# huangnengCSU/NanoSNP

Measured on NVIDIA B200. Metric: candidate sites/sec (s1+s2), higher is better.
Workload: dtype int32 counts, fp64 AF gate, fp16 hi/lo split x3 tensor-core model (fp32 accumulate)

## Files before the change

### nanosnp_b200/csrc/model_tc.cu

```cuda
#include <cuda_fp16.h>
#include <stdlib.h>
#include "model_common.cuh"
#include "tc_ptx.cuh"

namespace nsnp {
namespace {

constexpr int kRows = 128;
constexpr float kLog2e = 1.4426950408889634f;

__device__ __forceinline__ uint4 scale_hi(const uint4& hi) {
    const __half2 k = __float2half2_rn(1.0f / kTcLoScale);
    auto m = [&](uint32_t x) { __half2 t = *reinterpret_cast<__half2*>(&x); return h2_bits(__hmul2(t, k)); };
    return make_uint4(m(hi.x), m(hi.y), m(hi.z), m(hi.w));
}

template <int LAYER> struct TcCfg;
template <> struct TcCfg<0> { static constexpr int K = kTcK0, IN = kTcIn0, STEPS = 33; };
template <> struct TcCfg<1> { static constexpr int K = kTcK1, IN = kTcIn1, STEPS = 17; };

template <int LAYER, int CG> struct TcSmem {
    static constexpr int K = TcCfg<LAYER>::K;
    static constexpr int RB = 256 / CG;
    static constexpr size_t b_bytes = (size_t)K * RB * 2;
    static constexpr size_t a_bytes = (size_t)K * kRows * 2;
    static constexpr size_t sc_bytes = LAYER == 0 ? (size_t)kTcIn0 * kRows * 2 : 0;
    static constexpr size_t off_bhi = 0, off_blo = b_bytes, off_ahi = 2 * b_bytes, off_alo = off_ahi + a_bytes,
                            off_asc = off_alo + a_bytes, off_bar = off_asc + sc_bytes, off_bias = off_bar + 64,
                            total = off_bias + (LAYER == 1 ? 256 * sizeof(float) : 0);
};

template <int LAYER, int CG, int NWQ, bool DEBUG>
__global__ void __launch_bounds__(128 * NWQ + (LAYER == 1 ? 32 : 0), (LAYER == 0 && CG == 2 && NWQ == 2) ? 2 : 1)
lstm_tc_kernel(const unsigned char* __restrict__ blob, const int32_t* __restrict__ xi, const float* __restrict__ xf,
               const __half* __restrict__ h0_in, __half* __restrict__ h0_out, float* __restrict__ h16, float* __restrict__ dbg,
               int64_t n, int dir_override)
{
    using C = TcCfg<LAYER>;
    using S = TcSmem<LAYER, CG>;
    constexpr int K = C::K, IN = C::IN, RB = S::RB;
    constexpr int KB = K / 16;
    constexpr int kThreads = 128 * NWQ + (LAYER == 1 ? 32 : 0);
    constexpr int kEpiWarps = 4 * NWQ;
    constexpr int UB = 8 / NWQ;
    constexpr uint32_t LBO_A = kRows * 16, LBO_B = RB * 16, SBO = 128;
    extern __shared__ __align__(1024) unsigned char smem[];
    unsigned char* sBhi = smem + S::off_bhi; unsigned char* sBlo = smem + S::off_blo;
    unsigned char* sAhi = smem + S::off_ahi; unsigned char* sAlo = smem + S::off_alo; unsigned char* sAsc = smem + S::off_asc;
    uint64_t* bar = reinterpret_cast<uint64_t*>(smem + S::off_bar);
    uint32_t* tmem_slot = reinterpret_cast<uint32_t*>(smem + S::off_bar + 32);

    const int tid = threadIdx.x, lane = tid & 31, warp = tid >> 5;
    const bool producer = LAYER == 1 && warp == kEpiWarps;
    const int quad = warp & 3, sub = producer ? 0 : (warp >> 2);
    const int row = quad * 32 + lane;
    const int dir = DEBUG ? dir_override : (int)blockIdx.y;
    const uint32_t cta_rank = CG == 2 ? cluster_ctarank() : 0u;
    const int64_t site0 = (int64_t)blockIdx.x * kRows;
    int64_t site = site0 + row;
    const bool live = site < n;
    if (!live) site = n - 1;

    if (tid == 0) { mbar_init(bar, 1); mbar_init(bar + 1, 1); mbar_init(bar + 2, 1); fence_mbar_init(); }
    if (warp == 0) tmem_alloc<CG>(tmem_slot, LAYER == 1 ? 512 : 256);
    {
        const uint4* ghi = reinterpret_cast<const uint4*>(blob + tc_off(LAYER, dir, 0));
        const uint4* glo = reinterpret_cast<const uint4*>(blob + tc_off(LAYER, dir, 1));
        uint4* dhi = reinterpret_cast<uint4*>(sBhi); uint4* dlo = reinterpret_cast<uint4*>(sBlo);
        for (int i = tid; i < (K / 8) * RB; i += kThreads) {
            const int ch = i / RB, r = i - ch * RB;
            const int g = ch * 256 + (int)cta_rank * RB + r;
            dhi[i] = __ldg(ghi + g); dlo[i] = __ldg(glo + g);
        }
        uint4* a = reinterpret_cast<uint4*>(sAhi);
        const int n16 = (int)((2 * S::a_bytes + S::sc_bytes) / 16);
        for (int i = tid; i < n16; i += kThreads) a[i] = make_uint4(0, 0, 0, 0);
    }
    __syncthreads();
    const float* sBias = reinterpret_cast<const float*>(smem + S::off_bias);
    if (LAYER == 1) {
        const float* gb = reinterpret_cast<const float*>(blob + kOffTcBias1) + dir * 256;
        for (int i = tid; i < 256; i += kThreads) reinterpret_cast<float*>(smem + S::off_bias)[i] = __ldg(gb + i);
        __syncthreads();
    }

    float c[UB][8];
#pragma unroll
    for (int j = 0; j < UB; ++j)
#pragma unroll
        for (int u = 0; u < 8; ++u) c[j][u] = 0.f;

    int2 xraw[8];
    auto load_x = [&](int t) {
        if (LAYER != 0) return;
        const int2* g = reinterpret_cast<const int2*>(xi ? (const void*)(xi + (site * kT + t) * kF) : (const void*)(xf + (site * kT + t) * kF));
        if (sub == 0) {
#pragma unroll
            for (int j = 0; j < 8; ++j) xraw[j] = ldg_nc_volatile(g + j);
        } else if (sub == NWQ - 1) {
            xraw[0] = ldg_nc_volatile(g + 8);
        }
    };
    auto xval = [&](int j) -> float {
        const int2 p = xraw[j >> 1];
        const int b = (j & 1) ? p.y : p.x;
        return xi ? (float)b : __int_as_float(b);
    };
    auto store_x = [&]() {
        if (LAYER != 0) return;
        if (sub == 0) {
#pragma unroll
            for (int ch = 0; ch < 2; ++ch) {
                float v[8];
#pragma unroll
                for (int j = 0; j < 8; ++j) v[j] = xval(ch * 8 + j);
                const HiLo8 s = split8(v);
                reinterpret_cast<uint4*>(sAhi + ch * LBO_A)[row] = s.hi;
                reinterpret_cast<uint4*>(sAlo + ch * LBO_A)[row] = s.lo;
                reinterpret_cast<uint4*>(sAsc + ch * LBO_A)[row] = scale_hi(s.hi);
            }
        } else if (sub == NWQ - 1) {
            const float v[8] = {xval(0), xval(1), 1.0f, 0.f, 0.f, 0.f, 0.f, 0.f};
            const HiLo8 s = split8(v);
            reinterpret_cast<uint4*>(sAhi + 2 * LBO_A)[row] = s.hi;
            reinterpret_cast<uint4*>(sAlo + 2 * LBO_A)[row] = s.lo;
            reinterpret_cast<uint4*>(sAsc + 2 * LBO_A)[row] = scale_hi(s.hi);
        }
    };
    uint64_t* barS = bar + 2;
    constexpr uint32_t kPartBytes = 16u * kRows * 16u;
    const bool l2_prefetch = (dir_override >> 8) & 1;
    const int npass = ((dir_override >> 16) & 3) ? ((dir_override >> 16) & 3) : 3;
    const size_t src_tile = min((size_t)blockIdx.x, (size_t)((n + kRows - 1) / kRows - 1));
    auto stage_h0_bulk = [&](int t) {
        const __half* src = h0_in + (src_tile * kT + t) * (2 * kPartBytes / 2);
        mbar_expect_tx(barS, 2 * kPartBytes);
        bulk_g2s(sAhi, src, kPartBytes, barS);
        bulk_g2s(sAlo, src + kPartBytes / 2, kPartBytes, barS);
        const int tp = dir == 0 ? t + 1 : t - 1;
        if (l2_prefetch && tp >= 0 && tp < kT) bulk_prefetch_l2(h0_in + (src_tile * kT + tp) * (2 * kPartBytes / 2), 2 * kPartBytes);
    };
    constexpr int XB = IN / 16;
    constexpr uint32_t kTmemCols = LAYER == 1 ? 512 : 256;
    uint64_t* barH = bar;
    uint64_t* barX = bar + 1;
    {
        const int t0 = dir == 0 ? 0 : kT - 1;
        load_x(t0); store_x();
        fence_async_smem();
    }

    tc_fence_before();
    if (CG == 2) cluster_sync_all(); else __syncthreads();
    tc_fence_after();
    uint32_t phaseH = 0, phaseX = 0, phaseS = 0;
    if (LAYER == 1) {
        if (producer && lane == 0) stage_h0_bulk(dir == 0 ? 0 : kT - 1);
        mbar_wait(barS, phaseS); phaseS ^= 1;
        tc_fence_before();
        if (CG == 2) cluster_sync_all(); else __syncthreads();
        tc_fence_after();
    }
    const uint32_t tmem_base = *tmem_slot;
    const uint32_t a_hi = smem_u32(sAhi), a_lo = smem_u32(sAlo), a_sc = smem_u32(sAsc), b_hi = smem_u32(sBhi), b_lo = smem_u32(sBlo);
    constexpr uint32_t idesc = make_idesc(128 * CG, 256);
    const bool issuer = cta_rank == 0 && tid == 0;
    auto issue = [&](int kb0, int kb1, uint32_t tmem_d, uint32_t acc) {
#pragma unroll 1
        for (int pass = 0; pass < npass; ++pass) {
#pragma unroll 1
            for (int kb = kb0; kb < kb1; ++kb) {
                uint32_t aa = pass == 2 ? a_lo : a_hi;
                if (LAYER == 0 && pass == 1 && kb < kTcIn0 / 16) aa = a_sc;
                const uint32_t bb = pass == 1 ? b_lo : b_hi;
                umma_f16<CG>(tmem_d, make_desc(aa + kb * 2 * LBO_A, LBO_A, SBO), make_desc(bb + kb * 2 * LBO_B, LBO_B, SBO), idesc, acc);
                acc = 1;
            }
        }
    };
    if (LAYER == 1) {
        if (issuer) { tc_fence_after(); issue(0, XB, tmem_base, 0); umma_commit<CG>(barX); }
        if (producer) {
            mbar_wait(barX, phaseX); phaseX ^= 1;
            if (lane == 0 && C::STEPS > 1 && !DEBUG) stage_h0_bulk(dir == 0 ? 1 : kT - 2);
        }
    }

    for (int step = 0; step < C::STEPS; ++step) {
        const int t = dir == 0 ? step : (kT - 1 - step);
        const int tn = dir == 0 ? step + 1 : (kT - 2 - step);
        const bool more = !DEBUG && step + 1 < C::STEPS;
        const uint32_t acc_cols = LAYER == 1 ? (uint32_t)(step & 1) * 256u : 0u;
        if (LAYER == 1 && more) { mbar_wait(barS, phaseS); phaseS ^= 1; }
        fence_async_smem();
        tc_fence_before();
        if (CG == 2) cluster_sync_exec(); else __syncthreads();
        if (issuer) {
            tc_fence_after();
            if (LAYER == 1) {
                issue(XB, KB, tmem_base + acc_cols, 1);
                umma_commit<CG>(barH);
                if (more) { issue(0, XB, tmem_base + (acc_cols ^ 256u), 0); umma_commit<CG>(barX); }
            } else {
                issue(0, KB, tmem_base, 0);
                umma_commit<CG>(barH);
            }
        }
        if (producer) {
            if (more) {
                mbar_wait(barX, phaseX); phaseX ^= 1;
                if (lane == 0 && step + 2 < C::STEPS) stage_h0_bulk(dir == 0 ? step + 2 : kT - 3 - step);
            }
            if (DEBUG) break;
            continue;
        }
        if (more) load_x(tn);
        mbar_wait(barH, phaseH);
        phaseH ^= 1;
        tc_fence_after();

        if (DEBUG) {
#pragma unroll 1
            for (int jb = sub * UB; jb < sub * UB + UB; ++jb) {
                float v[32];
                tmem_ld32(tmem_base + acc_cols + ((uint32_t)(quad * 32) << 16) + jb * 32, v);
                if (live) for (int i = 0; i < 32; ++i) dbg[(site0 + row) * 256 + jb * 32 + i] = v[i] + (LAYER == 1 ? sBias[jb * 32 + i] : 0.f);
            }
            break;
        }

        uint32_t vb[2][16];
        const uint32_t tacc = tmem_base + acc_cols + ((uint32_t)(quad * 32) << 16) + (uint32_t)(sub * UB) * 32u;
        tmem_ld16_nowait(tacc, vb[0]);
        tmem_wait_ld();
        float hv[8];
#pragma unroll
        for (int hb = 0; hb < 2 * UB; ++hb) {
            const int jl = hb >> 1, uh = hb & 1, jb = sub * UB + jl;
            if (hb + 1 < 2 * UB) tmem_ld16_nowait(tacc + (hb + 1) * 16, vb[(hb + 1) & 1]);
#pragma unroll
            for (int u = 0; u < 4; ++u) {
                const uint32_t* v = vb[hb & 1];
                const float* bq = sBias + jb * 32 + uh * 16 + u;
                const float bi_ = LAYER == 1 ? bq[0] : 0.f, bf_ = LAYER == 1 ? bq[4] : 0.f, bg_ = LAYER == 1 ? bq[8] : 0.f, bo_ = LAYER == 1 ? bq[12] : 0.f;
                const float xi_ = fminf(__uint_as_float(v[u]) + bi_, 36.f), xf_ = fminf(__uint_as_float(v[4 + u]) + bf_, 36.f);
                const float xg_ = fminf(__uint_as_float(v[8 + u]) + bg_, 36.f), xo_ = __uint_as_float(v[12 + u]) + bo_;
                const float ei = ex2_approx(xi_), ef = ex2_approx(xf_), eg = ex2_approx(xg_), eo = ex2_approx(xo_);
                const float pi = 1.f + ei, pf = 1.f + ef, pg = 1.f + eg;
                const float pig = pi * pg;
                const float num = fmaf(c[jl][uh * 4 + u], pig, fmaf(eg, 2.f * kLog2e, -2.f * kLog2e) * pf);
                const float cn = num * rcp_approx(pf * pig);
                c[jl][uh * 4 + u] = cn;
                const float ec = ex2_approx(cn);
                hv[uh * 4 + u] = (1.f - ec) * rcp_approx((1.f + eo) * (1.f + ec));
            }
            if (hb + 1 < 2 * UB) tmem_wait_ld();
            if (uh == 1) {
                const HiLo8 s = split8(hv);
                reinterpret_cast<uint4*>(sAhi + (IN / 8 + jb) * LBO_A)[row] = s.hi;
                reinterpret_cast<uint4*>(sAlo + (IN / 8 + jb) * LBO_A)[row] = s.lo;
                if (live) {
                    if (LAYER == 0) {
                        __half* o = h0_out + ((((size_t)blockIdx.x * kT + t) * 2) * 16 + (dir * 8 + jb)) * (kRows * 8) + row * 8;
                        *reinterpret_cast<uint4*>(o) = s.hi;
                        *reinterpret_cast<uint4*>(o + 16 * kRows * 8) = s.lo;
                    } else if (step == C::STEPS - 1) {
                        float4* o = reinterpret_cast<float4*>(h16 + site * 128 + dir * kH + jb * 8);
                        o[0] = make_float4(hv[0], hv[1], hv[2], hv[3]); o[1] = make_float4(hv[4], hv[5], hv[6], hv[7]);
                    }
                }
            }
        }
        if (more) store_x();
    }

    tc_fence_before();
    if (CG == 2) cluster_sync_all(); else __syncthreads();
    if (warp == 0) tmem_dealloc<CG>(tmem_base, kTmemCols);
}


__device__ __forceinline__ void mbar_arrive(uint64_t* bar) {
    asm volatile("mbarrier.arrive.shared::cta.b64 _, [%0];" ::"r"(smem_u32(bar)) : "memory");
}

constexpr int kP2GroupThreads = 256, kP2Threads = 2 * kP2GroupThreads;
struct P2Smem {
    static constexpr size_t b_bytes = (size_t)kTcK0 * 128 * 2;
    static constexpr size_t a_bytes = (size_t)kTcK0 * kRows * 2;
    static constexpr size_t sc_bytes = (size_t)kTcIn0 * kRows * 2;
    static constexpr size_t a_stride = 2 * a_bytes + sc_bytes;
    static constexpr size_t off_bhi = 0, off_blo = b_bytes, off_a = 2 * b_bytes, off_bar = off_a + 2 * a_stride, total = off_bar + 128;
};

__global__ void __launch_bounds__(kP2Threads, 1)
lstm0_pair2_kernel(const unsigned char* __restrict__ blob, const int32_t* __restrict__ xi, const float* __restrict__ xf,
                   __half* __restrict__ h0_out, int64_t n, const int32_t* __restrict__ pos, int64_t pos_bias, int npass)
{
    using S = P2Smem;
// ... 325 lines not shown
                const float xi_ = fminf(__uint_as_float(v[u]) + bq[0], 36.f), xf_ = fminf(__uint_as_float(v[4 + u]) + bq[4], 36.f);
                const float xg_ = fminf(__uint_as_float(v[8 + u]) + bq[8], 36.f), xo_ = __uint_as_float(v[12 + u]) + bq[12];
                const float ei = ex2_approx(xi_), ef = ex2_approx(xf_), eg = ex2_approx(xg_), eo = ex2_approx(xo_);
                const float pi = 1.f + ei, pf = 1.f + ef, pg = 1.f + eg;
                const float pig = pi * pg;
                const float num = fmaf(c[jl][uh * 4 + u], pig, fmaf(eg, 2.f * kLog2e, -2.f * kLog2e) * pf);
                const float cn = num * rcp_approx(pf * pig);
                c[jl][uh * 4 + u] = cn;
                const float ec = ex2_approx(cn);
                hv[uh * 4 + u] = (1.f - ec) * rcp_approx((1.f + eo) * (1.f + ec));
            }
            if (hb + 1 < 2 * UB) tmem_wait_ld();
            if (uh == 1) {
                const HiLo8 sp = split8(hv);
                reinterpret_cast<uint4*>(sA + (IN / 8 + jb) * LBO_A)[row] = sp.hi;
                if (live && step == kS - 1) {
                    float4* o = reinterpret_cast<float4*>(h16 + site * 128 + dir * kH + jb * 8);
                    o[0] = make_float4(hv[0], hv[1], hv[2], hv[3]); o[1] = make_float4(hv[4], hv[5], hv[6], hv[7]);
                }
            }
        }
        if (more) {
            if (warp == 0) { mbar_wait(barIn, phaseIn); phaseIn ^= 1; }
            report_ready();
        }
        if (++step == kS) { step = 0; ++qi; }
    }

    tc_fence_before();
    cluster_sync_all();
    if (threadIdx.x < 32) tmem_dealloc<2>(*tmem_slot, 512);
}

template <class Kern, class... Args>
int launch_pair2(Kern kern, const char* name, size_t smem_bytes, int64_t m, cudaStream_t stream, Args... args) {
    const unsigned quads = (unsigned)((m + 4 * kRows - 1) / (4 * kRows));
    unsigned clusters = 2 * quads; if (clusters > (unsigned)kNumSMs / 2) clusters = ((unsigned)kNumSMs / 2) & ~1u;
    cudaLaunchConfig_t cfg = {};
    cfg.gridDim = dim3(2 * clusters, 1, 1);
    cfg.blockDim = dim3(kP2Threads, 1, 1);
    cfg.dynamicSmemBytes = smem_bytes;
    cfg.stream = stream;
    cudaLaunchAttribute attr[1];
    attr[0].id = cudaLaunchAttributeClusterDimension;
    attr[0].val.clusterDim.x = 2; attr[0].val.clusterDim.y = 1; attr[0].val.clusterDim.z = 1;
    cfg.attrs = attr; cfg.numAttrs = 1;
    const cudaError_t e = cudaLaunchKernelEx(&cfg, kern, args...);
    if (e != cudaSuccess) return set_error(NSNP_E_CUDA, "%s: %s", name, cudaGetErrorString(e));
    return NSNP_OK;
}

int launch_l0_pair2(const void* blob, const int32_t* xi, const float* xf, void* h0_out, int64_t m, const int32_t* pos, int64_t pos_bias, int npass, cudaStream_t stream) {
    static bool attr_done = false;
    if (!attr_done) {
        if (cudaFuncSetAttribute(lstm0_pair2_kernel, cudaFuncAttributeMaxDynamicSharedMemorySize, (int)P2Smem::total) != cudaSuccess)
            return cuda_status("cudaFuncSetAttribute(lstm0_pair2_kernel)");
        attr_done = true;
    }
    return launch_pair2(lstm0_pair2_kernel, "lstm0_pair2_kernel", P2Smem::total, m, stream, (const unsigned char*)blob, xi, xf, (__half*)h0_out, m, pos, pos_bias, npass);
}

int launch_l1_pair2(const void* blob, const void* h0_in, float* h16, int64_t m, cudaStream_t stream) {
    static bool attr_done = false;
    if (!attr_done) {
        if (cudaFuncSetAttribute(lstm1_pair2_kernel, cudaFuncAttributeMaxDynamicSharedMemorySize, (int)P2Smem1::total) != cudaSuccess)
            return cuda_status("cudaFuncSetAttribute(lstm1_pair2_kernel)");
        attr_done = true;
    }
    return launch_pair2(lstm1_pair2_kernel, "lstm1_pair2_kernel", P2Smem1::total, m, stream, (const unsigned char*)blob, (const __half*)h0_in, h16, m);
}

constexpr int kTtEpiWarps = 8, kTtLoadWarps = 4;
constexpr int kTtThreads = (kTtEpiWarps + kTtLoadWarps + 1) * 32;
struct TailSmem {
    static constexpr size_t w_bytes = kTcBytesTail;
    static constexpr size_t a_bytes = (size_t)128 * kRows * 2;
    static constexpr size_t off_whi = 0, off_wlo = w_bytes, off_ahi = 2 * w_bytes, off_alo = off_ahi + a_bytes,
                            off_head = off_alo + a_bytes,
                            off_bias = off_head + 256 * 24 * 4,
                            off_xch = off_bias + (256 + 32) * 4,
                            off_bar = off_xch + 128 * 12 * 4, total = off_bar + 64;
};

__device__ __forceinline__ void named_bar_sync(int id, int nthreads) { asm volatile("bar.sync %0, %1;" ::"r"(id), "r"(nthreads) : "memory"); }

__global__ void __launch_bounds__(kTtThreads, 1)
tail_tc_kernel(const unsigned char* __restrict__ blob, const float* __restrict__ h16, int64_t n_max, const int32_t* __restrict__ n_dev,
               float* __restrict__ gt, float* __restrict__ zy)
{
    using S = TailSmem;
    constexpr uint32_t LBO_A = kRows * 16, LBO_B = 256 * 16, SBO = 128;
    extern __shared__ __align__(1024) unsigned char smem[];
    unsigned char* sWhi = smem + S::off_whi; unsigned char* sWlo = smem + S::off_wlo;
    unsigned char* sAhi = smem + S::off_ahi; unsigned char* sAlo = smem + S::off_alo;
    float* sHead = reinterpret_cast<float*>(smem + S::off_head);
    float* sBias = reinterpret_cast<float*>(smem + S::off_bias);
    float* sXch = reinterpret_cast<float*>(smem + S::off_xch);
    uint64_t* bar = reinterpret_cast<uint64_t*>(smem + S::off_bar);
    uint32_t* tmem_slot = reinterpret_cast<uint32_t*>(smem + S::off_bar + 48);
    uint64_t* barH = bar; uint64_t* barIn = bar + 2; uint64_t* barFree = bar + 3;

    const int tid = threadIdx.x, lane = tid & 31, warp = tid >> 5;
// ... 131 lines not shown
            if (half == 0 && site < n) {
                float m = lg[0];
#pragma unroll
                for (int j = 1; j < 21; ++j) m = fmaxf(m, lg[j]);
                float sum = 0.f;
#pragma unroll
                for (int j = 0; j < 21; ++j) { lg[j] = expf(lg[j] - m); sum += lg[j]; }
#pragma unroll
                for (int j = 0; j < 21; ++j) gt[site * 21 + j] = lg[j] / sum;
                const float m2 = fmaxf(lg[21], fmaxf(lg[22], lg[23]));
                const float e0 = expf(lg[21] - m2), e1 = expf(lg[22] - m2), e2 = expf(lg[23] - m2);
                const float s2 = e0 + e1 + e2;
                zy[site * 3 + 0] = e0 / s2; zy[site * 3 + 1] = e1 / s2; zy[site * 3 + 2] = e2 / s2;
            }
        }
    }

    tc_fence_before();
    __syncthreads();
    if (warp == 0) tmem_dealloc<1>(tmem_base, 512);
}

template <int LAYER, int CG, int NWQ, bool DEBUG>
int launch_one(const void* blob, const int32_t* xi, const float* xf, const void* h0_in, void* h0_out, float* h16, float* dbg,
               int64_t m, int dir_override, cudaStream_t stream)
{
    using S = TcSmem<LAYER, CG>;
    auto kern = lstm_tc_kernel<LAYER, CG, NWQ, DEBUG>;
    static bool attr_done = false;
    if (!attr_done) {
        if (cudaFuncSetAttribute(kern, cudaFuncAttributeMaxDynamicSharedMemorySize, (int)S::total) != cudaSuccess) return cuda_status("cudaFuncSetAttribute(lstm_tc_kernel)");
        attr_done = true;
    }
    unsigned gx = (unsigned)((m + kRows - 1) / kRows);
    if (CG == 2 && (gx & 1)) ++gx;
    cudaLaunchConfig_t cfg = {};
    cfg.gridDim = dim3(gx, DEBUG ? 1 : 2, 1);
    cfg.blockDim = dim3(128 * NWQ + (LAYER == 1 ? 32 : 0), 1, 1);
    cfg.dynamicSmemBytes = S::total;
    cfg.stream = stream;
    cudaLaunchAttribute attr[1];
    attr[0].id = cudaLaunchAttributeClusterDimension;
    attr[0].val.clusterDim.x = CG; attr[0].val.clusterDim.y = 1; attr[0].val.clusterDim.z = 1;
    cfg.attrs = attr; cfg.numAttrs = 1;
    const cudaError_t e = cudaLaunchKernelEx(&cfg, kern, (const unsigned char*)blob, xi, xf, (const __half*)h0_in, (__half*)h0_out, h16, dbg, m, dir_override);
    if (e != cudaSuccess) return set_error(NSNP_E_CUDA, "lstm_tc_kernel<%d,%d,%d>: %s", LAYER, CG, NWQ, cudaGetErrorString(e));
    return NSNP_OK;
}

}

int launch_tail_tc(const void* blob, const float* h16, int64_t n_max, const int32_t* n_dev, float* gt, float* zy, cudaStream_t stream) {
    using S = TailSmem;
    static bool attr_done = false;
    if (!attr_done) {
        if (cudaFuncSetAttribute(tail_tc_kernel, cudaFuncAttributeMaxDynamicSharedMemorySize, (int)S::total) != cudaSuccess)
            return cuda_status("cudaFuncSetAttribute(tail_tc_kernel)");
        attr_done = true;
    }
    const int64_t n_tiles = (n_max + kRows - 1) / kRows;
    const int grid = (int)(n_tiles < kNumSMs ? n_tiles : kNumSMs);
    tail_tc_kernel<<<grid, kTtThreads, S::total, stream>>>((const unsigned char*)blob, h16, n_max, n_dev, gt, zy);
    return cuda_status("tail_tc_kernel");
}

int launch_lstm_tc(const void* blob, const int32_t* xi, const float* xf, void* h0, float* h16, int64_t m, const int32_t* pos, int64_t pos_bias, int npass, cudaStream_t stream) {
    {
        ProfScope prof(NSNP_PROF_LSTM0, stream);
        static const int variant = [] { const char* v = getenv("NSNP_L0_VARIANT"); return v ? atoi(v) : 1; }();
        if (pos && variant != 1) return set_error(NSNP_E_UNSUPPORTED, "window reads from the count tensor need the default layer-0 kernel");
        if (int e = variant == 1 ? launch_l0_pair2(blob, xi, xf, h0, m, pos, pos_bias, npass, stream)
                                 : launch_one<0, 2, 2, false>(blob, xi, xf, nullptr, h0, nullptr, nullptr, m, npass << 16, stream)) return e;
    }
    ProfScope prof(NSNP_PROF_LSTM1, stream);
    static const int pf = [] { const char* v = getenv("NSNP_L1_PREFETCH"); return v ? atoi(v) : 1; }();
    static const int l1_variant = [] { const char* v = getenv("NSNP_L1_VARIANT"); return v ? atoi(v) : 1; }();
    if (npass == 1 && l1_variant == 1) return launch_l1_pair2(blob, h0, h16, m, stream);
    return launch_one<1, 2, 4, false>(blob, nullptr, nullptr, h0, nullptr, h16, nullptr, m, (pf << 8) | (npass << 16), stream);
}

int debug_tc_gates(const void* blob, const int32_t* xi, int layer, int dir, int cg, const void* h0, float* gates_out, int64_t m, cudaStream_t stream) {
    if (layer == 0 && cg == 1) return launch_one<0, 1, 2, true>(blob, xi, nullptr, nullptr, nullptr, nullptr, gates_out, m, dir, stream);
    if (layer == 0 && cg == 2) return launch_one<0, 2, 2, true>(blob, xi, nullptr, nullptr, nullptr, nullptr, gates_out, m, dir, stream);
    if (layer == 1 && cg == 2) return launch_one<1, 2, 4, true>(blob, nullptr, nullptr, h0, nullptr, nullptr, gates_out, m, dir, stream);
    return set_error(NSNP_E_UNSUPPORTED, "debug_tc_gates: layer %d with cta_group %d is not built", layer, cg);
}

int pack_tc_weights(const nsnp_model_weights_t* w, unsigned char* blob) {
    for (int layer = 0; layer < 2; ++layer) {
        const int K = layer == 0 ? kTcK0 : kTcK1, IN = layer == 0 ? kTcIn0 : kTcIn1, nin = layer == 0 ? kF : 128;
        for (int d = 0; d < 2; ++d) {
            __half* hi = reinterpret_cast<__half*>(blob + tc_off(layer, d, 0));
            __half* lo = reinterpret_cast<__half*>(blob + tc_off(layer, d, 1));
            const float *wih = w->w_ih[layer][d], *whh = w->w_hh[layer][d], *bi = w->b_ih[layer][d], *bh = w->b_hh[layer][d];
            for (int n = 0; n < 256; ++n) {
                const int jb = n >> 5, uh = (n >> 4) & 1, gate = (n >> 2) & 3, u4 = n & 3;
                const int rowi = gate * kH + jb * 8 + uh * 4 + u4;
                for (int k = 0; k < K; ++k) {
                    float v = 0.f;
                    if (k < nin) v = wih[rowi * nin + k];
                    else if (layer == 0 && k == nin) v = bi[rowi] + bh[rowi];
                    else if (k >= IN) v = whh[rowi * kH + (k - IN)];
                    v *= gate == 2 ? -2.0f * kLog2e : -kLog2e;
                    const float scale = (layer == 0 && k < IN) ? kTcLoScale : 1.0f;
                    const __half h = __float2half_rn(v);
                    const __half l = __float2half_rn((v - __half2float(h)) * scale);
                    const size_t idx = ((size_t)(k >> 3) * 256 + n) * 8 + (k & 7);
                    hi[idx] = h; lo[idx] = l;
                }
                if (layer == 1) reinterpret_cast<float*>(blob + kOffTcBias1)[d * 256 + n] = (bi[rowi] + bh[rowi]) * (gate == 2 ? -2.0f * kLog2e : -kLog2e);
// ... 28 lines not shown
```

### nanosnp_b200/csrc/tc_ptx.cuh

```cuda
#pragma once
#include <cuda_fp16.h>
#include <stdint.h>

namespace nsnp {
namespace {

__device__ __forceinline__ uint32_t smem_u32(const void* p) { return (uint32_t)__cvta_generic_to_shared(p); }
__device__ __forceinline__ void mbar_init(uint64_t* bar, uint32_t count) {
    asm volatile("mbarrier.init.shared::cta.b64 [%0], %1;" ::"r"(smem_u32(bar)), "r"(count) : "memory");
}
__device__ __forceinline__ void fence_mbar_init() { asm volatile("fence.mbarrier_init.release.cluster;" ::: "memory"); }
__device__ __forceinline__ void mbar_wait(uint64_t* bar, uint32_t parity) {
    asm volatile(
        "{\n\t.reg .pred P1;\n\t"
        "WAIT_LOOP:\n\t"
        "mbarrier.try_wait.parity.shared::cta.b64 P1, [%0], %1;\n\t"
        "@P1 bra DONE;\n\t"
        "bra WAIT_LOOP;\n\t"
        "DONE:\n\t}"
        ::"r"(smem_u32(bar)), "r"(parity) : "memory");
}
__device__ __forceinline__ void mbar_wait_cluster(uint64_t* bar, uint32_t parity) {
    asm volatile(
        "{\n\t.reg .pred P1;\n\t"
        "WAIT_LOOP_C:\n\t"
        "mbarrier.try_wait.parity.acquire.cluster.shared::cta.b64 P1, [%0], %1;\n\t"
        "@P1 bra DONE_C;\n\t"
        "bra WAIT_LOOP_C;\n\t"
        "DONE_C:\n\t}"
        ::"r"(smem_u32(bar)), "r"(parity) : "memory");
}
__device__ __forceinline__ void mbar_arrive_remote_relaxed(uint64_t* bar, uint32_t target_cta) {
    uint32_t raddr;
    asm volatile("mapa.shared::cluster.u32 %0, %1, %2;" : "=r"(raddr) : "r"(smem_u32(bar)), "r"(target_cta));
    asm volatile("mbarrier.arrive.relaxed.cluster.shared::cluster.b64 _, [%0];" ::"r"(raddr) : "memory");
}
__device__ __forceinline__ void fence_async_smem() { asm volatile("fence.proxy.async.shared::cta;" ::: "memory"); }
__device__ __forceinline__ void tc_fence_before() { asm volatile("tcgen05.fence::before_thread_sync;" ::: "memory"); }
__device__ __forceinline__ void tc_fence_after() { asm volatile("tcgen05.fence::after_thread_sync;" ::: "memory"); }
__device__ __forceinline__ void cluster_sync_all() {
    asm volatile("barrier.cluster.arrive.release.aligned;\n\tbarrier.cluster.wait.acquire.aligned;" ::: "memory");
}
__device__ __forceinline__ void cluster_sync_exec() {
    asm volatile("barrier.cluster.arrive.relaxed.aligned;\n\tbarrier.cluster.wait.aligned;" ::: "memory");
}
__device__ __forceinline__ uint32_t cluster_ctarank() { uint32_t r; asm volatile("mov.u32 %0, %%cluster_ctarank;" : "=r"(r)); return r; }

template <int CG> __device__ __forceinline__ void tmem_alloc(uint32_t* dst_smem, uint32_t ncols) {
    if (CG == 1) {
        asm volatile("tcgen05.alloc.cta_group::1.sync.aligned.shared::cta.b32 [%0], %1;" ::"r"(smem_u32(dst_smem)), "r"(ncols) : "memory");
        asm volatile("tcgen05.relinquish_alloc_permit.cta_group::1.sync.aligned;" ::: "memory");
    } else {
        asm volatile("tcgen05.alloc.cta_group::2.sync.aligned.shared::cta.b32 [%0], %1;" ::"r"(smem_u32(dst_smem)), "r"(ncols) : "memory");
        asm volatile("tcgen05.relinquish_alloc_permit.cta_group::2.sync.aligned;" ::: "memory");
    }
}
template <int CG> __device__ __forceinline__ void tmem_dealloc(uint32_t taddr, uint32_t ncols) {
    if (CG == 1) asm volatile("tcgen05.dealloc.cta_group::1.sync.aligned.b32 %0, %1;" ::"r"(taddr), "r"(ncols) : "memory");
    else asm volatile("tcgen05.dealloc.cta_group::2.sync.aligned.b32 %0, %1;" ::"r"(taddr), "r"(ncols) : "memory");
}
template <int CG> __device__ __forceinline__ void umma_f16(uint32_t tmem_d, uint64_t adesc, uint64_t bdesc, uint32_t idesc, uint32_t accumulate) {
    if (CG == 1)
        asm volatile("{\n\t.reg .pred p;\n\tsetp.ne.b32 p, %4, 0;\n\ttcgen05.mma.cta_group::1.kind::f16 [%0], %1, %2, %3, p;\n\t}"
                     ::"r"(tmem_d), "l"(adesc), "l"(bdesc), "r"(idesc), "r"(accumulate) : "memory");
    else
        asm volatile("{\n\t.reg .pred p;\n\tsetp.ne.b32 p, %4, 0;\n\ttcgen05.mma.cta_group::2.kind::f16 [%0], %1, %2, %3, p;\n\t}"
                     ::"r"(tmem_d), "l"(adesc), "l"(bdesc), "r"(idesc), "r"(accumulate) : "memory");
}
// ... 79 lines not shown
```

Measured before the change: 41.58 million.

## Make layer-1 LSTM kernel persistent with cross-tile pipelined input GEMM and cluster barrier

Layer 1 now launches a persistent grid capped at the SM count. Each cluster loops over several 128-row tiles for one direction and resets the cell state at each tile boundary. The h0 bulk staging and the input-projection MMA are pipelined across tile boundaries, so the next tile's first step overlaps with the current tile's last step. A new cluster-scope mbarrier lets the rank-0 issuer, now the producer warp, wait until both CTAs have staged their inputs. This is meant to remove per-tile launch, TMEM allocation and weight-load overhead and to keep the tensor core busy. The cost is more complex phase tracking and fewer resident CTAs when there are few tiles.

Result: faster. 42.08 million, median of 6 (+1.2%).

```diff
diff --git a/nanosnp_b200/csrc/model_tc.cu b/nanosnp_b200/csrc/model_tc.cu
--- a/nanosnp_b200/csrc/model_tc.cu
+++ b/nanosnp_b200/csrc/model_tc.cu
@@ -40,6 +40,7 @@
     using S = TcSmem<LAYER, CG>;
     constexpr int K = C::K, IN = C::IN, RB = S::RB;
     constexpr int KB = K / 16;
+    constexpr int kS = DEBUG ? 1 : C::STEPS;
     constexpr int kThreads = 128 * NWQ + (LAYER == 1 ? 32 : 0);
     constexpr int kEpiWarps = 4 * NWQ;
     constexpr int UB = 8 / NWQ;
@@ -54,14 +55,31 @@
     const bool producer = LAYER == 1 && warp == kEpiWarps;
     const int quad = warp & 3, sub = producer ? 0 : (warp >> 2);
     const int row = quad * 32 + lane;
-    const int dir = DEBUG ? dir_override : (int)blockIdx.y;
     const uint32_t cta_rank = CG == 2 ? cluster_ctarank() : 0u;
-    const int64_t site0 = (int64_t)blockIdx.x * kRows;
-    int64_t site = site0 + row;
-    const bool live = site < n;
-    if (!live) site = n - 1;
-
-    if (tid == 0) { mbar_init(bar, 1); mbar_init(bar + 1, 1); mbar_init(bar + 2, 1); fence_mbar_init(); }
+    int dir, unit0, unit_stride = 0, my_tiles = 1;
+    if (LAYER == 1) {
+        const int cluster = (int)blockIdx.x / CG, n_clusters = (int)gridDim.x / CG;
+        const int n_units = (int)((n + CG * kRows - 1) / (CG * kRows));
+        dir = DEBUG ? dir_override : cluster & 1;
+        unit0 = DEBUG ? cluster : cluster >> 1;
+        unit_stride = DEBUG ? n_clusters : n_clusters >> 1;
+        my_tiles = (n_units - unit0 + unit_stride - 1) / unit_stride;
+    } else {
+        dir = DEBUG ? dir_override : (int)blockIdx.y;
+        unit0 = (int)blockIdx.x / CG;
+    }
+    const int total = my_tiles * kS;
+    auto tile_of = [&](int qi) -> int64_t { return (int64_t)(unit0 + qi * unit_stride) * CG + cta_rank; };
+    int64_t tile = LAYER == 1 ? tile_of(0) : (int64_t)blockIdx.x, site;
+    bool live;
+    auto enter_tile = [&]() {
+        site = tile * kRows + row;
+        live = site < n;
+        if (!live) site = n - 1;
+    };
+    enter_tile();
+
+    if (tid == 0) { mbar_init(bar, 1); mbar_init(bar + 1, 1); mbar_init(bar + 2, 1); mbar_init(bar + 3, CG); fence_mbar_init(); }
     if (warp == 0) tmem_alloc<CG>(tmem_slot, LAYER == 1 ? 512 : 256);
     {
         const uint4* ghi = reinterpret_cast<const uint4*>(blob + tc_off(LAYER, dir, 0));
@@ -84,12 +102,6 @@
         __syncthreads();
     }
 
-    float c[UB][8];
-#pragma unroll
-    for (int j = 0; j < UB; ++j)
-#pragma unroll
-        for (int u = 0; u < 8; ++u) c[j][u] = 0.f;
-
     int2 xraw[8];
     auto load_x = [&](int t) {
         if (LAYER != 0) return;
@@ -131,19 +143,23 @@
     constexpr uint32_t kPartBytes = 16u * kRows * 16u;
     const bool l2_prefetch = (dir_override >> 8) & 1;
     const int npass = ((dir_override >> 16) & 3) ? ((dir_override >> 16) & 3) : 3;
-    const size_t src_tile = min((size_t)blockIdx.x, (size_t)((n + kRows - 1) / kRows - 1));
-    auto stage_h0_bulk = [&](int t) {
-        const __half* src = h0_in + (src_tile * kT + t) * (2 * kPartBytes / 2);
+    auto h0_rows = [&](int e) -> const __half* {
+        if (e >= total) return nullptr;
+        const int qi = e / kS, st = e - qi * kS;
+        const size_t src_tile = min((size_t)tile_of(qi), (size_t)((n + kRows - 1) / kRows - 1));
+        return h0_in + (src_tile * kT + (dir == 0 ? st : kT - 1 - st)) * (2 * kPartBytes / 2);
+    };
+    auto stage_h0_bulk = [&](const __half* src, const __half* next) {
         mbar_expect_tx(barS, 2 * kPartBytes);
         bulk_g2s(sAhi, src, kPartBytes, barS);
         bulk_g2s(sAlo, src + kPartBytes / 2, kPartBytes, barS);
-        const int tp = dir == 0 ? t + 1 : t - 1;
-        if (l2_prefetch && tp >= 0 && tp < kT) bulk_prefetch_l2(h0_in + (src_tile * kT + tp) * (2 * kPartBytes / 2), 2 * kPartBytes);
+        if (l2_prefetch && next) bulk_prefetch_l2(next, 2 * kPartBytes);
     };
     constexpr int XB = IN / 16;
     constexpr uint32_t kTmemCols = LAYER == 1 ? 512 : 256;
     uint64_t* barH = bar;
     uint64_t* barX = bar + 1;
+    uint64_t* barIn = bar + 3;
     {
         const int t0 = dir == 0 ? 0 : kT - 1;
         load_x(t0); store_x();
@@ -153,10 +169,9 @@
     tc_fence_before();
     if (CG == 2) cluster_sync_all(); else __syncthreads();
     tc_fence_after();
-    uint32_t phaseH = 0, phaseX = 0, phaseS = 0;
     if (LAYER == 1) {
-        if (producer && lane == 0) stage_h0_bulk(dir == 0 ? 0 : kT - 1);
-        mbar_wait(barS, phaseS); phaseS ^= 1;
+        if (producer && lane == 0) stage_h0_bulk(h0_rows(0), h0_rows(1));
+        mbar_wait(barS, 0);
         tc_fence_before();
         if (CG == 2) cluster_sync_all(); else __syncthreads();
         tc_fence_after();
@@ -164,7 +179,7 @@
     const uint32_t tmem_base = *tmem_slot;
     const uint32_t a_hi = smem_u32(sAhi), a_lo = smem_u32(sAlo), a_sc = smem_u32(sAsc), b_hi = smem_u32(sBhi), b_lo = smem_u32(sBlo);
     constexpr uint32_t idesc = make_idesc(128 * CG, 256);
-    const bool issuer = cta_rank == 0 && tid == 0;
+    const bool issuer = cta_rank == 0 && tid == (LAYER == 1 ? kEpiWarps * 32 : 0);
     auto issue = [&](int kb0, int kb1, uint32_t tmem_d, uint32_t acc) {
 #pragma unroll 1
         for (int pass = 0; pass < npass; ++pass) {
@@ -181,42 +196,52 @@
     if (LAYER == 1) {
         if (issuer) { tc_fence_after(); issue(0, XB, tmem_base, 0); umma_commit<CG>(barX); }
         if (producer) {
-            mbar_wait(barX, phaseX); phaseX ^= 1;
-            if (lane == 0 && C::STEPS > 1 && !DEBUG) stage_h0_bulk(dir == 0 ? 1 : kT - 2);
-        }
-    }
-
-    for (int step = 0; step < C::STEPS; ++step) {
-        const int t = dir == 0 ? step : (kT - 1 - step);
-        const int tn = dir == 0 ? step + 1 : (kT - 2 - step);
-        const bool more = !DEBUG && step + 1 < C::STEPS;
-        const uint32_t acc_cols = LAYER == 1 ? (uint32_t)(step & 1) * 256u : 0u;
-        if (LAYER == 1 && more) { mbar_wait(barS, phaseS); phaseS ^= 1; }
+            mbar_wait(barX, 0);
+            if (lane == 0 && total > 1) stage_h0_bulk(h0_rows(1), h0_rows(2));
+        }
+    }
+
+    float c[UB][8];
+    for (int g = 0; g < total; ++g) {
+        const int qi = LAYER == 1 ? g / kS : 0, st = g - qi * kS;
+        const int t = dir == 0 ? st : (kT - 1 - st);
+        const int tn = dir == 0 ? st + 1 : (kT - 2 - st);
+        const bool more = g + 1 < total;
+        const uint32_t acc_cols = LAYER == 1 ? (uint32_t)(g & 1) * 256u : 0u;
+        if (st == 0) {
+            if (g > 0) { tile = tile_of(qi); enter_tile(); }
+#pragma unroll
+            for (int j = 0; j < UB; ++j)
+#pragma unroll
+                for (int u = 0; u < 8; ++u) c[j][u] = 0.f;
+        }
         fence_async_smem();
         tc_fence_before();
         if (CG == 2) cluster_sync_exec(); else __syncthreads();
-        if (issuer) {
-            tc_fence_after();
-            if (LAYER == 1) {
-                issue(XB, KB, tmem_base + acc_cols, 1);
-                umma_commit<CG>(barH);
-                if (more) { issue(0, XB, tmem_base + (acc_cols ^ 256u), 0); umma_commit<CG>(barX); }
-            } else {
-                issue(0, KB, tmem_base, 0);
-                umma_commit<CG>(barH);
-            }
-        }
-        if (producer) {
+        if (LAYER == 0) {
+            if (issuer) { tc_fence_after(); issue(0, KB, tmem_base, 0); umma_commit<CG>(barH); }
+        } else if (producer) {
+            if (issuer) { tc_fence_after(); issue(XB, KB, tmem_base + acc_cols, 1); umma_commit<CG>(barH); }
             if (more) {
-                mbar_wait(barX, phaseX); phaseX ^= 1;
-                if (lane == 0 && step + 2 < C::STEPS) stage_h0_bulk(dir == 0 ? step + 2 : kT - 3 - step);
-            }
-            if (DEBUG) break;
+                const __half* src = h0_rows(g + 2);
+                const __half* next = h0_rows(g + 3);
+                if (lane == 0) {
+                    mbar_wait(barS, (uint32_t)(g + 1) & 1u);
+                    mbar_arrive_remote_release(barIn, 0);
+                }
+                if (issuer) {
+                    mbar_wait_cluster(barIn, (uint32_t)g & 1u);
+                    tc_fence_after();
+                    issue(0, XB, tmem_base + (acc_cols ^ 256u), 0);
+                    umma_commit<CG>(barX);
+                }
+                mbar_wait(barX, (uint32_t)(g + 1) & 1u);
+                if (lane == 0 && src) stage_h0_bulk(src, next);
+            }
             continue;
         }
         if (more) load_x(tn);
-        mbar_wait(barH, phaseH);
-        phaseH ^= 1;
+        mbar_wait(barH, (uint32_t)g & 1u);
         tc_fence_after();
 
         if (DEBUG) {
@@ -224,9 +249,9 @@
             for (int jb = sub * UB; jb < sub * UB + UB; ++jb) {
                 float v[32];
                 tmem_ld32(tmem_base + acc_cols + ((uint32_t)(quad * 32) << 16) + jb * 32, v);
-                if (live) for (int i = 0; i < 32; ++i) dbg[(site0 + row) * 256 + jb * 32 + i] = v[i] + (LAYER == 1 ? sBias[jb * 32 + i] : 0.f);
-            }
-            break;
+                if (live) for (int i = 0; i < 32; ++i) dbg[site * 256 + jb * 32 + i] = v[i] + (LAYER == 1 ? sBias[jb * 32 + i] : 0.f);
+            }
+            continue;
         }
 
         uint32_t vb[2][16];
@@ -257,14 +282,15 @@
             if (hb + 1 < 2 * UB) tmem_wait_ld();
             if (uh == 1) {
                 const HiLo8 s = split8(hv);
-                reinterpret_cast<uint4*>(sAhi + (IN / 8 + jb) * LBO_A)[row] = s.hi;
-                reinterpret_cast<uint4*>(sAlo + (IN / 8 + jb) * LBO_A)[row] = s.lo;
+                const bool h_zero = LAYER == 1 && st == kS - 1;
+                reinterpret_cast<uint4*>(sAhi + (IN / 8 + jb) * LBO_A)[row] = h_zero ? make_uint4(0, 0, 0, 0) : s.hi;
+                reinterpret_cast<uint4*>(sAlo + (IN / 8 + jb) * LBO_A)[row] = h_zero ? make_uint4(0, 0, 0, 0) : s.lo;
                 if (live) {
                     if (LAYER == 0) {
-                        __half* o = h0_out + ((((size_t)blockIdx.x * kT + t) * 2) * 16 + (dir * 8 + jb)) * (kRows * 8) + row * 8;
+                        __half* o = h0_out + ((((size_t)tile * kT + t) * 2) * 16 + (dir * 8 + jb)) * (kRows * 8) + row * 8;
                         *reinterpret_cast<uint4*>(o) = s.hi;
                         *reinterpret_cast<uint4*>(o + 16 * kRows * 8) = s.lo;
-                    } else if (step == C::STEPS - 1) {
+                    } else if (st == kS - 1) {
                         float4* o = reinterpret_cast<float4*>(h16 + site * 128 + dir * kH + jb * 8);
                         o[0] = make_float4(hv[0], hv[1], hv[2], hv[3]); o[1] = make_float4(hv[4], hv[5], hv[6], hv[7]);
                     }
@@ -889,10 +915,16 @@
         if (cudaFuncSetAttribute(kern, cudaFuncAttributeMaxDynamicSharedMemorySize, (int)S::total) != cudaSuccess) return cuda_status("cudaFuncSetAttribute(lstm_tc_kernel)");
         attr_done = true;
     }
-    unsigned gx = (unsigned)((m + kRows - 1) / kRows);
+    unsigned gx = (unsigned)((m + kRows - 1) / kRows), gy = DEBUG ? 1 : 2;
     if (CG == 2 && (gx & 1)) ++gx;
+    if (LAYER == 1) {
+        const unsigned units = gx / CG, cap = ((unsigned)kNumSMs / CG) & ~1u;
+        unsigned clusters = DEBUG ? units : 2 * units;
+        if (clusters > cap) clusters = cap;
+        gx = clusters * CG; gy = 1;
+    }
     cudaLaunchConfig_t cfg = {};
-    cfg.gridDim = dim3(gx, DEBUG ? 1 : 2, 1);
+    cfg.gridDim = dim3(gx, gy, 1);
     cfg.blockDim = dim3(128 * NWQ + (LAYER == 1 ? 32 : 0), 1, 1);
     cfg.dynamicSmemBytes = S::total;
     cfg.stream = stream;
diff --git a/nanosnp_b200/csrc/tc_ptx.cuh b/nanosnp_b200/csrc/tc_ptx.cuh
--- a/nanosnp_b200/csrc/tc_ptx.cuh
+++ b/nanosnp_b200/csrc/tc_ptx.cuh
@@ -34,6 +34,11 @@
     uint32_t raddr;
     asm volatile("mapa.shared::cluster.u32 %0, %1, %2;" : "=r"(raddr) : "r"(smem_u32(bar)), "r"(target_cta));
     asm volatile("mbarrier.arrive.relaxed.cluster.shared::cluster.b64 _, [%0];" ::"r"(raddr) : "memory");
+}
+__device__ __forceinline__ void mbar_arrive_remote_release(uint64_t* bar, uint32_t target_cta) {
+    uint32_t raddr;
+    asm volatile("mapa.shared::cluster.u32 %0, %1, %2;" : "=r"(raddr) : "r"(smem_u32(bar)), "r"(target_cta));
+    asm volatile("mbarrier.arrive.release.cluster.shared::cluster.b64 _, [%0];" ::"r"(raddr) : "memory");
 }
 __device__ __forceinline__ void fence_async_smem() { asm volatile("fence.proxy.async.shared::cta;" ::: "memory"); }
 __device__ __forceinline__ void tc_fence_before() { asm volatile("tcgen05.fence::before_thread_sync;" ::: "memory"); }
```

## Add warp-specialized paired-CTA layer-1 LSTM kernel for three-pass hi/lo split

Applied to the files above, without the earlier changes.

Adds a new layer-1 LSTM kernel for the three-pass (hi/lo split) path. It uses 2-CTA clusters and a dedicated producer warp that streams hi and lo input halves through separate full/empty mbarriers, and it ping-pongs two tile groups on the tensor core. Before this, the npass==3 case fell back to the generic launch_one kernel. The aim is to overlap input loading and the recurrent epilogue with UMMA work and to share weights across the CTA pair. In exchange it adds considerable synchronization complexity, and the input buffer is single-buffered per half, which may stall.

New measurement: 41.15 million before, 43.34 million after, median of 6. +5.3%, better.

```diff
diff --git a/nanosnp_b200/csrc/model_tc.cu b/nanosnp_b200/csrc/model_tc.cu
--- a/nanosnp_b200/csrc/model_tc.cu
+++ b/nanosnp_b200/csrc/model_tc.cu
@@ -656,13 +656,234 @@
     if (threadIdx.x < 32) tmem_dealloc<2>(*tmem_slot, 512);
 }
 
+constexpr int kP2x3Threads = kP2Threads + 32;
+struct P2Smem1x3 {
+    static constexpr size_t b_bytes = (size_t)kTcK1 * 128 * 2;
+    static constexpr size_t in_bytes = (size_t)kTcIn1 * kRows * 2;
+    static constexpr size_t h_bytes = (size_t)kH * kRows * 2;
+    static constexpr size_t off_bhi = 0, off_blo = b_bytes, off_in = 2 * b_bytes, off_h = off_in + 2 * in_bytes,
+                            off_bias = off_h + 4 * h_bytes, off_bar = off_bias + 256 * sizeof(float), total = off_bar + 128;
+};
+static_assert(P2Smem1x3::total <= 232448, "lstm1_pair2x3_kernel: shared memory above the per-block opt-in limit");
+
+__global__ void __launch_bounds__(kP2x3Threads, 1)
+lstm1_pair2x3_kernel(const unsigned char* __restrict__ blob, const __half* __restrict__ h0_in, float* __restrict__ h16, int64_t n)
+{
+    using S = P2Smem1x3;
+    constexpr int K = kTcK1, IN = kTcIn1, KB = K / 16, XB = IN / 16, RB = 128, UB = 4, kS = TcCfg<1>::STEPS;
+    constexpr uint32_t LBO_A = kRows * 16, LBO_B = RB * 16, SBO = 128;
+    constexpr uint32_t kPartBytes = 16u * kRows * 16u;
+    extern __shared__ __align__(1024) unsigned char smem[];
+    const bool producer = threadIdx.x >= kP2Threads;
+    const int grp = producer ? 0 : (int)threadIdx.x / kP2GroupThreads;
+    const int tid = (int)threadIdx.x - grp * kP2GroupThreads, lane = tid & 31, warp = tid >> 5;
+    unsigned char* sBhi = smem + S::off_bhi; unsigned char* sBlo = smem + S::off_blo;
+    unsigned char* sInHi = smem + S::off_in; unsigned char* sInLo = sInHi + S::in_bytes;
+    unsigned char* sHhi = smem + S::off_h + grp * 2 * S::h_bytes; unsigned char* sHlo = sHhi + S::h_bytes;
+    float* sBias = reinterpret_cast<float*>(smem + S::off_bias);
+    uint64_t* bars = reinterpret_cast<uint64_t*>(smem + S::off_bar);
+    uint64_t* barH = bars + grp;
+    uint64_t* barReady = bars + 2 + grp;
+    uint64_t* barTurn = bars + 4;
+    uint64_t* barHiFull = bars + 6;
+    uint64_t* barLoFull = bars + 8;
+    uint64_t* barHiEmpty = bars + 10;
+    uint64_t* barLoEmpty = bars + 11;
+    uint32_t* tmem_slot = reinterpret_cast<uint32_t*>(smem + S::off_bar + 96);
+
+    const int quad = warp & 3, sub = warp >> 2;
+    const int row = quad * 32 + lane;
+    const uint32_t cta_rank = cluster_ctarank();
+    const int cluster_id = (int)(blockIdx.x >> 1);
+    const int dir = cluster_id & 1;
+    const int quad_stride = (int)(gridDim.x >> 2);
+    const int n_quads = (int)((n + 4 * kRows - 1) / (4 * kRows));
+    const int64_t last_tile = (n + kRows - 1) / kRows - 1;
+    const int q0 = cluster_id >> 1;
+    const int my_quads = q0 < n_quads ? (n_quads - q0 + quad_stride - 1) / quad_stride : 0;
+    const int total_g = my_quads * kS;
+    auto tile_of = [&](int qi, int g) -> int64_t { return (int64_t)(q0 + qi * quad_stride) * 4 + (int64_t)cta_rank * 2 + g; };
+
+    if (threadIdx.x == 0) {
+        mbar_init(bars + 0, 1); mbar_init(bars + 1, 1); mbar_init(bars + 2, 16); mbar_init(bars + 3, 16);
+        for (int i = 4; i < 12; ++i) mbar_init(bars + i, 1);
+        fence_mbar_init();
+    }
+    if (threadIdx.x < 32) tmem_alloc<2>(tmem_slot, 512);
+    {
+        const uint4* ghi = reinterpret_cast<const uint4*>(blob + tc_off(1, dir, 0));
+        const uint4* glo = reinterpret_cast<const uint4*>(blob + tc_off(1, dir, 1));
+        uint4* dhi = reinterpret_cast<uint4*>(sBhi); uint4* dlo = reinterpret_cast<uint4*>(sBlo);
+        for (int i = (int)threadIdx.x; i < (K / 8) * RB; i += kP2x3Threads) {
+            const int ch = i / RB, r = i - ch * RB;
+            const int g = ch * 256 + (int)cta_rank * RB + r;
+            dhi[i] = __ldg(ghi + g); dlo[i] = __ldg(glo + g);
+        }
+        const float* gb = reinterpret_cast<const float*>(blob + kOffTcBias1) + dir * 256;
+        for (int i = (int)threadIdx.x; i < 256; i += kP2x3Threads) sBias[i] = __ldg(gb + i);
+    }
+    __syncthreads();
+
+    auto rows_of = [&](int b) -> const __half* {
+        const int gs = b >> 1, qi = gs / kS, st = gs - qi * kS;
+        const int t = dir == 0 ? st : (kT - 1 - st);
+        const int64_t tile = min(tile_of(qi, b & 1), last_tile);
+        return h0_in + ((size_t)tile * kT + t) * (size_t)kPartBytes;
+    };
+    const int total_b = 2 * total_g;
+    if (producer && lane == 0 && total_b > 0) {
+        const __half* src = rows_of(0);
+        mbar_expect_tx(barHiFull, kPartBytes); bulk_g2s(sInHi, src, kPartBytes, barHiFull);
+        mbar_expect_tx(barLoFull, kPartBytes); bulk_g2s(sInLo, src + kPartBytes / 2, kPartBytes, barLoFull);
+        if (total_b > 1) bulk_prefetch_l2(rows_of(1), 2 * kPartBytes);
+    }
+    auto report_ready = [&]() {
+        fence_async_smem();
+        tc_fence_before();
+        __syncwarp();
+        if (lane == 0) mbar_arrive_remote_relaxed(barReady, 0);
+    };
+    uint32_t phaseIn = 0;
+    auto wait_input = [&]() {
+        mbar_wait(barHiFull + grp, phaseIn);
+        mbar_wait(barLoFull + grp, phaseIn);
+        phaseIn ^= 1;
+    };
+    tc_fence_before();
+    cluster_sync_all();
+    tc_fence_after();
+
+    if (producer) {
+        if (lane == 0) {
+            for (int b = 1; b < total_b; ++b) {
+                const __half* src = rows_of(b);
+                uint64_t* full_hi = barHiFull + (b & 1); uint64_t* full_lo = barLoFull + (b & 1);
+                mbar_wait(barHiEmpty, (uint32_t)((b - 1) & 1));
+                mbar_expect_tx(full_hi, kPartBytes); bulk_g2s(sInHi, src, kPartBytes, full_hi);
+                if (b + 1 < total_b) bulk_prefetch_l2(rows_of(b + 1), 2 * kPartBytes);
+                mbar_wait(barLoEmpty, (uint32_t)((b - 1) & 1));
+                mbar_expect_tx(full_lo, kPartBytes); bulk_g2s(sInLo, src + kPartBytes / 2, kPartBytes, full_lo);
+            }
+        }
+        __syncwarp();
+    } else {
+        float c[UB][8];
+#pragma unroll
+        for (int j = 0; j < UB; ++j)
+#pragma unroll
+            for (int u = 0; u < 8; ++u) c[j][u] = 0.f;
+
+        if (total_g > 0) {
+            if (warp == 0) wait_input();
+            report_ready();
+        }
+
+        const uint32_t tmem_base = *tmem_slot + (uint32_t)grp * 256u;
+        const uint32_t in_hi = smem_u32(sInHi), in_lo = smem_u32(sInLo), h_hi = smem_u32(sHhi), h_lo = smem_u32(sHlo);
+        const uint32_t b_hi = smem_u32(sBhi), b_lo = smem_u32(sBlo);
+        constexpr uint32_t idesc = make_idesc(256, 256);
+        const bool issuer = cta_rank == 0 && tid == 0;
+        uint32_t phaseH = 0, phaseR = 0, phaseT = 0;
+        if (cta_rank == 0 && threadIdx.x == 0) mbar_arrive(barTurn + 0);
+
+        int step = 0, qi = 0;
+        for (int g = 0; g < total_g; ++g) {
+            const bool more = g + 1 < total_g;
+            const int64_t site = tile_of(qi, grp) * kRows + row;
+            const bool live = site < n;
+            float* const out = h16 + site * 128 + dir * kH + sub * UB * 8;
+            if (step == 0) {
+#pragma unroll
+                for (int j = 0; j < UB; ++j)
+#pragma unroll
+                    for (int u = 0; u < 8; ++u) c[j][u] = 0.f;
+            }
+            if (issuer) {
+                const bool refill = more || grp == 0;
+                mbar_wait_cluster(barReady, phaseR);
+                mbar_wait(barTurn + grp, phaseT);
+                tc_fence_after();
+#pragma unroll 1
+                for (int pass = 0; pass < 3; ++pass) {
+#pragma unroll 1
+                    for (int kb = 0; kb < XB; ++kb)
+                        umma_f16<2>(tmem_base, make_desc((pass == 2 ? in_lo : in_hi) + kb * 2 * LBO_A, LBO_A, SBO),
+                                    make_desc((pass == 1 ? b_lo : b_hi) + kb * 2 * LBO_B, LBO_B, SBO), idesc, (pass | kb) ? 1u : 0u);
+                    if (pass == 1 && refill) umma_commit<2>(barHiEmpty);
+                }
+                if (refill) umma_commit<2>(barLoEmpty);
+                if (step > 0) {
+#pragma unroll 1
+                    for (int pass = 0; pass < 3; ++pass) {
+#pragma unroll 1
+                        for (int kb = XB; kb < KB; ++kb)
+                            umma_f16<2>(tmem_base, make_desc((pass == 2 ? h_lo : h_hi) + (kb - XB) * 2 * LBO_A, LBO_A, SBO),
+                                        make_desc((pass == 1 ? b_lo : b_hi) + kb * 2 * LBO_B, LBO_B, SBO), idesc, 1u);
+                    }
+                }
+                umma_commit<2>(barH);
+                mbar_arrive(barTurn + (grp ^ 1));
+            }
+            phaseR ^= 1; phaseT ^= 1;
+            mbar_wait(barH, phaseH);
+            phaseH ^= 1;
+            tc_fence_after();
+
+            uint32_t vb[2][16];
+            const uint32_t tacc = tmem_base + ((uint32_t)(quad * 32) << 16) + (uint32_t)(sub * UB) * 32u;
+            tmem_ld16_nowait(tacc, vb[0]);
+            tmem_wait_ld();
+            float hv[8];
+#pragma unroll
+            for (int hb = 0; hb < 2 * UB; ++hb) {
+                const int jl = hb >> 1, uh = hb & 1, jb = sub * UB + jl;
+                if (hb + 1 < 2 * UB) tmem_ld16_nowait(tacc + (hb + 1) * 16, vb[(hb + 1) & 1]);
+#pragma unroll
+                for (int u = 0; u < 4; ++u) {
+                    const uint32_t* v = vb[hb & 1];
+                    const float* bq = sBias + jb * 32 + uh * 16 + u;
+                    const float xi_ = fminf(__uint_as_float(v[u]) + bq[0], 36.f), xf_ = fminf(__uint_as_float(v[4 + u]) + bq[4], 36.f);
+                    const float xg_ = fminf(__uint_as_float(v[8 + u]) + bq[8], 36.f), xo_ = __uint_as_float(v[12 + u]) + bq[12];
+                    const float ei = ex2_approx(xi_), ef = ex2_approx(xf_), eg = ex2_approx(xg_), eo = ex2_approx(xo_);
+                    const float pi = 1.f + ei, pf = 1.f + ef, pg = 1.f + eg;
+                    const float pig = pi * pg;
+                    const float num = fmaf(c[jl][uh * 4 + u], pig, fmaf(eg, 2.f * kLog2e, -2.f * kLog2e) * pf);
+                    const float cn = num * rcp_approx(pf * pig);
+                    c[jl][uh * 4 + u] = cn;
+                    const float ec = ex2_approx(cn);
+                    hv[uh * 4 + u] = (1.f - ec) * rcp_approx((1.f + eo) * (1.f + ec));
+                }
+                if (hb + 1 < 2 * UB) tmem_wait_ld();
+                if (uh == 1) {
+                    const HiLo8 sp = split8(hv);
+                    reinterpret_cast<uint4*>(sHhi + jb * LBO_A)[row] = sp.hi;
+                    reinterpret_cast<uint4*>(sHlo + jb * LBO_A)[row] = sp.lo;
+                    if (live && step == kS - 1) {
+                        float4* o = reinterpret_cast<float4*>(out + jl * 8);
+                        o[0] = make_float4(hv[0], hv[1], hv[2], hv[3]); o[1] = make_float4(hv[4], hv[5], hv[6], hv[7]);
+                    }
+                }
+            }
+            if (more) {
+                if (warp == 0) wait_input();
+                report_ready();
+            }
+            if (++step == kS) { step = 0; ++qi; }
+        }
+    }
+
+    tc_fence_before();
+    cluster_sync_all();
+    if (threadIdx.x < 32) tmem_dealloc<2>(*tmem_slot, 512);
+}
+
 template <class Kern, class... Args>
-int launch_pair2(Kern kern, const char* name, size_t smem_bytes, int64_t m, cudaStream_t stream, Args... args) {
+int launch_pair2(Kern kern, const char* name, size_t smem_bytes, int threads, int64_t m, cudaStream_t stream, Args... args) {
     const unsigned quads = (unsigned)((m + 4 * kRows - 1) / (4 * kRows));
     unsigned clusters = 2 * quads; if (clusters > (unsigned)kNumSMs / 2) clusters = ((unsigned)kNumSMs / 2) & ~1u;
     cudaLaunchConfig_t cfg = {};
     cfg.gridDim = dim3(2 * clusters, 1, 1);
-    cfg.blockDim = dim3(kP2Threads, 1, 1);
+    cfg.blockDim = dim3((unsigned)threads, 1, 1);
     cfg.dynamicSmemBytes = smem_bytes;
     cfg.stream = stream;
     cudaLaunchAttribute attr[1];
@@ -681,7 +902,7 @@
             return cuda_status("cudaFuncSetAttribute(lstm0_pair2_kernel)");
         attr_done = true;
     }
-    return launch_pair2(lstm0_pair2_kernel, "lstm0_pair2_kernel", P2Smem::total, m, stream, (const unsigned char*)blob, xi, xf, (__half*)h0_out, m, pos, pos_bias, npass);
+    return launch_pair2(lstm0_pair2_kernel, "lstm0_pair2_kernel", P2Smem::total, kP2Threads, m, stream, (const unsigned char*)blob, xi, xf, (__half*)h0_out, m, pos, pos_bias, npass);
 }
 
 int launch_l1_pair2(const void* blob, const void* h0_in, float* h16, int64_t m, cudaStream_t stream) {
@@ -691,7 +912,17 @@
             return cuda_status("cudaFuncSetAttribute(lstm1_pair2_kernel)");
         attr_done = true;
     }
-    return launch_pair2(lstm1_pair2_kernel, "lstm1_pair2_kernel", P2Smem1::total, m, stream, (const unsigned char*)blob, (const __half*)h0_in, h16, m);
+    return launch_pair2(lstm1_pair2_kernel, "lstm1_pair2_kernel", P2Smem1::total, kP2Threads, m, stream, (const unsigned char*)blob, (const __half*)h0_in, h16, m);
+}
+
+int launch_l1_pair2x3(const void* blob, const void* h0_in, float* h16, int64_t m, cudaStream_t stream) {
+    static bool attr_done = false;
+    if (!attr_done) {
+        if (cudaFuncSetAttribute(lstm1_pair2x3_kernel, cudaFuncAttributeMaxDynamicSharedMemorySize, (int)P2Smem1x3::total) != cudaSuccess)
+            return cuda_status("cudaFuncSetAttribute(lstm1_pair2x3_kernel)");
+        attr_done = true;
+    }
+    return launch_pair2(lstm1_pair2x3_kernel, "lstm1_pair2x3_kernel", P2Smem1x3::total, kP2x3Threads, m, stream, (const unsigned char*)blob, (const __half*)h0_in, h16, m);
 }
 
 constexpr int kTtEpiWarps = 8, kTtLoadWarps = 4;
@@ -933,6 +1164,7 @@
     static const int pf = [] { const char* v = getenv("NSNP_L1_PREFETCH"); return v ? atoi(v) : 1; }();
     static const int l1_variant = [] { const char* v = getenv("NSNP_L1_VARIANT"); return v ? atoi(v) : 1; }();
     if (npass == 1 && l1_variant == 1) return launch_l1_pair2(blob, h0, h16, m, stream);
+    if (npass == 3 && l1_variant == 1) return launch_l1_pair2x3(blob, h0, h16, m, stream);
     return launch_one<1, 2, 4, false>(blob, nullptr, nullptr, h0, nullptr, h16, nullptr, m, (pf << 8) | (npass << 16), stream);
 }
 
```
